# MrTornado24/FENeRF

Measured on AMD Instinct MI355X. Metric: rays/s/GPU forward render (128x128, 24+24 samples, H=256 FiLM-SIREN + 32x96^3 grid), higher is better.
Workload: dtype f16x3 (error-compensated fp16 MFMA, fp32 accumulate; fp32-class accuracy); 1 GPU; configs[1]: CelebA_double_semantic_texture_embedding_256_dim_96 generator, 128x128, 24+24 hierarchical samples, batch 1/GPU, forward-only render, procedural weights; img_size=128, num_steps=24, batch_per_gpu=1

## Files before the change

fenerf_amd/csrc/fenerf_api.cpp:

```cpp
#include <hip/hip_runtime.h>

#include <atomic>
#include <cstddef>
#include <cstdio>
#include <cstdlib>
#include <cstring>
#include <map>
#include <mutex>
#include <new>
#include <string>
#include <vector>

#include "fenerf_internal.h"

namespace fenerf {
static thread_local std::string g_err;
void set_error(const std::string& msg) { g_err = msg; }

static int fail(int code, const std::string& msg) {
  set_error(msg);
  return code;
}
static int hip_fail(hipError_t e, const char* what) {
  return fail(FENERF_E_HIP, std::string(what) + ": " + hipGetErrorString(e));
// ... 159 lines not shown
  {
    std::lock_guard<std::mutex> lock(g_phase_mu);
    recs.swap(g_phase_recs);
  }
  int rc = FENERF_OK;
  for (PhaseRec* r : recs) {
    float t = 0.f;
    hipError_t e = hipEventSynchronize(r->e1);
    if (e == hipSuccess) e = hipEventElapsedTime(&t, r->e0, r->e1);
    if (e == hipSuccess) { ms[r->phase] += (double)t; calls[r->phase] += 1; }
    else rc = hip_fail(e, "fenerf_phase_times");
    (void)hipEventDestroy(r->e0);
    (void)hipEventDestroy(r->e1);
    delete r;
  }
  return rc;
}
extern "C" int fenerf_abi_version(void) { return FENERF_ABI_VERSION; }
static thread_local int g_render_fusion = FENERF_FUSION_AUTO;
static constexpr bool kFusionAutoEnabled = false;
extern "C" int fenerf_set_render_fusion(int mode) {
  const int prev = g_render_fusion;
  g_render_fusion = (mode == FENERF_FUSION_OFF || mode == FENERF_FUSION_FORCE) ? mode : FENERF_FUSION_AUTO;
  return prev;
}
extern "C" int fenerf_set_cu_budget(int cus) {
  const int prev = g_cu_budget;
  g_cu_budget = cus > 0 ? cus : 0;
  return prev;
}

namespace {
struct FieldInfo { const char* name; long offset; };
struct StructInfo { const char* name; long size; const FieldInfo* fields; int n; };
#define FLD(S, f) {#f, (long)offsetof(S, f)}
const FieldInfo kDescFields[] = {
    FLD(FenerfModelDesc, abi_version), FLD(FenerfModelDesc, hidden_dim), FLD(FenerfModelDesc, n_geo), FLD(FenerfModelDesc, n_color),
    FLD(FenerfModelDesc, n_label_layers), FLD(FenerfModelDesc, output_dim), FLD(FenerfModelDesc, grid_ch), FLD(FenerfModelDesc, grid_d),
    FLD(FenerfModelDesc, grid_h), FLD(FenerfModelDesc, grid_w), FLD(FenerfModelDesc, box_scale), FLD(FenerfModelDesc, geo_w),
    FLD(FenerfModelDesc, geo_b), FLD(FenerfModelDesc, color_w), FLD(FenerfModelDesc, color_b), FLD(FenerfModelDesc, label_w),
    FLD(FenerfModelDesc, label_b), FLD(FenerfModelDesc, sigma_w), FLD(FenerfModelDesc, sigma_b), FLD(FenerfModelDesc, rgb_w),
    FLD(FenerfModelDesc, rgb_b), FLD(FenerfModelDesc, grid), FLD(FenerfModelDesc, precision), FLD(FenerfModelDesc, differentiable),
    FLD(FenerfModelDesc, wgrad_bf16_min_points)};
const FieldInfo kOptsFields[] = {
    FLD(FenerfCompositeOpts, clamp_mode), FLD(FenerfCompositeOpts, noise_std), FLD(FenerfCompositeOpts, last_back),
    FLD(FenerfCompositeOpts, white_back), FLD(FenerfCompositeOpts, black_back), FLD(FenerfCompositeOpts, fill_mode),
// ... 851 lines not shown
  p.rows_a = rows_a; p.rows_b = rows_b; p.z_a = z_a; p.z_b = z_b; p.noise = noise; p.o = *opts;
  p.g_rgb = g_rgb; p.d_rows_a = d_rows_a; p.d_rows_b = d_rows_b;
  { PhaseScope ph(PH_COMPOSITE_BWD, stream); return launch_composite_backward(p, merge != 0, stream); }
}

extern "C" size_t fenerf_sparse_select_workspace_bytes(int B, int64_t P) {
  if (B < 1 || P < 1) return 0;
  return sparse_select_workspace_bytes(B, P);
}

extern "C" int fenerf_sparse_select(int B, int R, int N, int C, int64_t cap, const float* d_coarse, const float* d_fine, const float* z_coarse,
                                    const float* z_fine, const float* origins, const float* dirs, const int64_t* images, float* pts, float* rd,
                                    float* d_sel, int32_t* counts, void* workspace, size_t workspace_bytes, void* stream) {
  if (B < 1 || B > 65535 || R < 1 || N < 1 || C < 1 || cap < 1) return fail(FENERF_E_INVALID, "need 1 <= B <= 65535, R, N, C, cap >= 1");
  if ((int64_t)R * N > (int64_t)1 << 36) return fail(FENERF_E_INVALID, "too many samples per image");
  if (!d_coarse || !z_coarse || !origins || !dirs || !pts || !d_sel || !counts || !workspace || (!d_fine) != (!z_fine))
    return fail(FENERF_E_INVALID, "NULL pointer (d_fine and z_fine may be NULL together: one pass)");
  if (workspace_bytes < sparse_select_workspace_bytes(B, (int64_t)R * N)) return fail(FENERF_E_INVALID, "workspace too small (fenerf_sparse_select_workspace_bytes)");
  { PhaseScope ph(PH_OTHER, stream); return launch_sparse_select(B, R, N, C, cap, d_coarse, d_fine, z_coarse, z_fine, origins, dirs, (const long long*)images, pts, rd, d_sel, counts, workspace, stream); }
}

namespace {
struct RenderWs {
  size_t film, coarse, fine, wts, zf, total;
};
RenderWs render_ws(const FenerfModel* m, int B, int R, int N, int hier) {
  RenderWs w;
  const size_t pts = (size_t)B * R * N;
  size_t off = 0;
  w.film = off; off += fenerf_film_workspace_bytes(m, B);
  w.coarse = off; off += align_up(pts * m->C * sizeof(float), 256);
  w.fine = off; off += hier ? align_up(pts * m->C * sizeof(float), 256) : 0;
  w.wts = off; off += hier ? align_up(pts * sizeof(float), 256) : 0;
  w.zf = off; off += hier ? align_up(pts * sizeof(float), 256) : 0;
  w.total = off;
  return w;
}
}

extern "C" size_t fenerf_render_workspace_bytes(const FenerfModel* m, int B, int R, int N, int hierarchical) {
  if (!m || B <= 0 || R <= 0 || N <= 0) return 0;
  return render_ws(m, B, R, N, hierarchical).total;
}

extern "C" int fenerf_render_forward(const FenerfModel* m, int B, int R, int N, int hierarchical, int lock_view,
                                     const float* origins, const float* dirs, const float* z_coarse, const float* u,
                                     const float* noise_coarse, const float* noise_final, const float* freq_geo,
                                     const float* phase_geo, const float* freq_app, const float* phase_app,
                                     const FenerfCompositeOpts* opts, float* out_rgb, float* out_depth,
                                     float* out_weights, float* out_wsum, void* workspace, size_t workspace_bytes,
                                     void* stream) {
  if (!m) return fail(FENERF_E_INVALID, "model is NULL");
  int rc = check_opts(opts);
  if (rc) return rc;
  if (B <= 0 || R <= 0 || N <= 0) return fail(FENERF_E_INVALID, "B, R, N must be > 0");
  const int M = hierarchical ? 2 * N : N;
  if (M > FENERF_MAX_RAY_SAMPLES) return fail(FENERF_E_INVALID, "at most 1024 samples per ray (512 + 512 hierarchical; FENERF_MAX_RAY_SAMPLES)");
// ... 30 lines not shown
    cp.out_ch = out_channels(m->C, opts);
    return run_composite(cp, false, stream);
  }
  float* fine = (float*)(base + ws.fine);
  float* zf = (float*)(base + ws.zf);
  FusedRenderPlan plan;
  if ((g_render_fusion == FENERF_FUSION_FORCE || (g_render_fusion == FENERF_FUSION_AUTO && kFusionAutoEnabled)) &&
      fused_render_plan(m, B, R, N, g_render_fusion == FENERF_FUSION_AUTO, &plan)) {
    CompositeParams c1, c2;
    memset(&c1, 0, sizeof(c1));
    c1.BR = BR; c1.M = N; c1.C = m->C; c1.N = N;
    c1.rows_a = coarse; c1.z_a = z_coarse; c1.noise = noise_coarse;
    c1.o.clamp_mode = opts->clamp_mode; c1.o.noise_std = opts->noise_std;
    c1.sigma_only = 1; c1.out_ch = m->C - 1;
    c1.u = u; c1.z_fine = zf;
    memset(&c2, 0, sizeof(c2));
    c2.BR = BR; c2.M = 2 * N; c2.C = m->C; c2.N = N;
    c2.rows_a = fine; c2.rows_b = coarse; c2.z_a = zf; c2.z_b = z_coarse; c2.noise = noise_final; c2.o = *opts;
    c2.out_rgb = out_rgb; c2.out_depth = out_depth; c2.out_weights = out_weights; c2.out_wsum = out_wsum;
    c2.out_ch = out_channels(m->C, opts);
    sp.out = coarse;
    PhaseScope ph(PH_RENDER_FUSED, stream);
    return launch_render16w_fused(m, sp, plan, zf, fine, c1, c2, stream);
  }
  rc = run_siren(m, sp, stream);
  if (rc) return rc;
  sp.raw_fg = nullptr;
  memset(&cp, 0, sizeof(cp));
  cp.BR = BR; cp.M = N; cp.C = m->C; cp.N = N;
  cp.rows_a = coarse; cp.z_a = z_coarse; cp.noise = noise_coarse;
  cp.o.clamp_mode = opts->clamp_mode; cp.o.noise_std = opts->noise_std;
  cp.sigma_only = 1; cp.out_ch = m->C - 1;
  cp.u = u; cp.z_fine = zf;
  rc = run_composite(cp, false, stream);
  if (rc) return rc;
  sp.z = zf; sp.out = fine;
  rc = run_siren(m, sp, stream);
  if (rc) return rc;
  memset(&cp, 0, sizeof(cp));
  cp.BR = BR; cp.M = 2 * N; cp.C = m->C; cp.N = N;
  cp.rows_a = fine; cp.rows_b = coarse; cp.z_a = zf; cp.z_b = z_coarse; cp.noise = noise_final; cp.o = *opts;
  cp.out_rgb = out_rgb; cp.out_depth = out_depth; cp.out_weights = out_weights; cp.out_wsum = out_wsum;
  cp.out_ch = out_channels(m->C, opts);
  return run_composite(cp, true, stream);
}

// ... 387 lines not shown
```

fenerf_amd/csrc/fenerf_internal.h:

```cpp
#pragma once
#include <cstddef>
#include <cstdint>
#include <map>
#include <mutex>
#include <string>
#include <vector>

#include "../../include/fenerf.h"
#include "fenerf_layout.h"

namespace fenerf {

void set_error(const std::string& msg);
int ensure_dynamic_lds(const void* kfn, size_t bytes);
enum Phase { PH_FILM_PREP = 0, PH_SIREN, PH_SIREN_SAVE, PH_CHAIN, PH_WGRAD_FILM, PH_WGRAD_SQ, PH_WGRAD_SQ_REDUCE, PH_WGRAD_THIN,
             PH_WGRAD_THIN_REDUCE, PH_COMPOSITE, PH_RESAMPLE, PH_COMPOSITE_BWD, PH_REPACK, PH_GRID, PH_RAY_SETUP, PH_OTHER, PH_RENDER_FUSED, PH_COUNT };
static_assert(PH_COUNT == FENERF_N_PHASES, "include/fenerf.h FENERF_N_PHASES");
struct PhaseScope {
  PhaseScope(int phase, void* stream);
  ~PhaseScope();
  void* rec;
};
int launch_cus(const FenerfModel* m);
int check_trig_domain();
// ... 41 lines not shown
  const float* grid;
  int gd, gh, gw;
  float box_scale;
  const float* points;
  const float* pdirs;
  const float* origins;
  const float* dirs;
  const float* z;
  int n_per_ray;
  int lock_view;
  long long P;
  long long pts_per_image;
  float* out;
  long long ring_offset_floats;
  float* tape;
  float* tape_e;
  int tape_format;
  int film_per_point;
  unsigned long long* clk;
  const float* raw_fg; const float* raw_pg; const float* raw_fa; const float* raw_pa;
  const float* film_bias;
  const float* film_inv_scale;
  int n_images;
};

struct SirenBwdParams {
  const float* stream;
  long long ring_offset_floats;
  const float* fp;
  const float* pp;
  long long P, pts_per_image;
  const float* out;
  const float* d_out;
  const float* tape;
  int tape_format;
  float* d_t;
  int bf16_dump;
  float* d_e;
  float* film_tiles;
  const float* points;
  float* d_grid_cl;
  float box_scale;
  int gd, gh, gw;
  int film_per_point;
};

// ... 15 lines not shown
  float* d_rows_a;
  float* d_rows_b;
};

int launch_film_prep(const FenerfModel* m, long long B, const float* fg, const float* pg, const float* fa, const float* pa,
                     float* fp, float* pp, void* stream, bool for_f32_kernel = false,
                     bool twice = false);
int launch_siren(const FenerfModel* m, const SirenParams& p, void* stream);
int launch_siren_f32(const FenerfModel* m, const SirenParams& p, void* stream);
int launch_siren_backward(const FenerfModel* m, const SirenBwdParams& p, void* stream);
int launch_siren_backward16w(const FenerfModel* m, const SirenBwdParams& p, void* stream);
bool use_bf16_dump(const FenerfModel* m, long long total_points);
int bwd16w_film_unit(long long total_points, long long pts_per_image);
size_t wgrad_workspace_bytes(const FenerfModel* m, int B, long long P);
int launch_param_grads(const FenerfModel* m, int B, long long P, const float* points, const float* dirs, const float* fp, const float* pp,
                       const float* out, const float* d_out, const float* tape, const float* tape_e, const float* d_t,
                       const FenerfSirenGrads& g, bool film_only, void* workspace, void* stream, const float* film_tiles = nullptr,
                       int tape_format = 0, const FenerfSirenGrads* weights = nullptr,
                       int film_per_point = 0);
int launch_grid_backward(const FenerfModel* m, long long P, const float* points, const float* d_e, float* d_grid_cl, void* stream);
int launch_siren_input_grads(const FenerfModel* m, int B, long long P, const float* points, const float* fp, const float* d_t, const float* w_geo0,
                             const float* w_color0, int w_color0_ld, float* d_points, float* d_dirs, void* stream);
int launch_siren16w(const FenerfModel* m, const SirenParams& p, void* stream);
struct FusedRenderPlan { int rays_per_group, octs_per_group, blocks; long long groups; };
bool fused_render_plan(const FenerfModel* m, long long B, long long R, int N, bool balanced_only, FusedRenderPlan* plan);
int launch_render16w_fused(const FenerfModel* m, const SirenParams& p, const FusedRenderPlan& plan, float* z_fine, float* out_fine,
                           const CompositeParams& coarse, const CompositeParams& final_, void* stream);
int launch_composite(const CompositeParams& p, bool merge, void* stream);
int launch_composite_backward(const CompositeParams& p, bool merge, void* stream);
int launch_resample(long long BR, int N, const float* z, const float* w, const float* u, float* zf, void* stream);
int launch_sample_pdf(long long BR, int K, int NS, const float* bins, const float* w, const float* u, float* out, void* stream);
int launch_ray_setup(int B, int S, int N, float z_cam, float ray_start, float ray_end, const float* u_jitter,
                     const float* theta, const float* phi, float* origins, float* dirs, float* z, float* pitch, float* yaw,
                     void* stream);
#define FENERF_MULTI_ADD_MAX 64
struct MultiAdd { float* dst[FENERF_MULTI_ADD_MAX]; const float* src[FENERF_MULTI_ADD_MAX]; long long n[FENERF_MULTI_ADD_MAX]; int count; };
struct FilmFold { float* out[4]; const float* in[4]; int row[4]; int B; };
int launch_render_points(int B, int R, int N, long long Pp, const float* origins, const float* dirs, const float* z, float* pts, float* rd, void* stream);
size_t sparse_select_workspace_bytes(int B, long long P);
int launch_sparse_select(int B, int R, int N, int C, long long cap, const float* d_coarse, const float* d_fine, const float* z_coarse,
                         const float* z_fine, const float* origins, const float* dirs, const long long* images, float* pts, float* rd, float* d_sel,
                         int* counts, void* workspace, void* stream);
int launch_pad_rows(const float* src, float* dst, long long nb, long long P, long long Pp, int C, bool to_padded, void* stream);
int launch_multi_add(const MultiAdd& J, void* stream);
int launch_film_fold(const FilmFold& J, void* stream);
int launch_repack(FenerfModel* m, const float* flat, const FenerfRepackMaps* r, float* scale_fwd, float* scale_bwd, void* stream);
// ... 5 lines not shown
```

fenerf_amd/csrc/fenerf_siren_f16w.hip:

```cpp
#include <hip/hip_runtime.h>

#include <type_traits>

#include "fenerf_composite_ray.h"
#include "fenerf_film.h"
#include "fenerf_internal.h"
#include "fenerf_layout.h"
#include "fenerf_trig.h"


namespace fenerf {
namespace w16 {

typedef float f32x4 __attribute__((ext_vector_type(4)));
typedef _Float16 half8 __attribute__((ext_vector_type(8)));
typedef _Float16 half4 __attribute__((ext_vector_type(4)));
typedef _Float16 half2 __attribute__((ext_vector_type(2)));

#define MFMA16W(a, b, c) __builtin_amdgcn_mfma_f32_16x16x32_f16((a), (b), (c), 0, 0, 0)
#define MFMA32W(a, b, c) __builtin_amdgcn_mfma_f32_16x16x4f32((a), (b), (c), 0, 0, 0)

constexpr int CH = FENERF_CH;
constexpr int DPF = FENERF_DPF;
constexpr int NSLOT = FENERF_NSLOT;
// ... 44 lines not shown
}
__device__ __forceinline__ void st_u4_nt(const void* g_uniform, unsigned voff, const u32x4& v) {
  asm volatile("global_store_dwordx4 %0, %1, %2 " FENERF_ST_POLICY "\n\ts_nop 1" : : "v"(voff), "v"(v), "s"(g_uniform) : "memory");
}
struct TapeQ { unsigned q[4]; };
__device__ __forceinline__ unsigned phase_u16(float theta) {
  return __builtin_bit_cast(unsigned, __builtin_fmaf(__builtin_amdgcn_fractf(theta), 65536.f, 8388608.f));
}
#define LDS_FENCE() asm volatile("" ::: "memory")
#ifndef FENERF_WAVE_HALF_COPIES
#define FENERF_WAVE_HALF_COPIES 1
#endif
#ifndef FENERF_EXP_DEPHASE
#define FENERF_EXP_DEPHASE 0
#endif

struct WStream {
  bool skip;
  unsigned long long g_next;
  unsigned voff;
  unsigned ring_lds;
  const char* ring_lane;
  bool early;
};

__device__ __forceinline__ void ws_issue(WStream& w, int slot) {
  const unsigned m0 = w.ring_lds + (unsigned)slot * (CH * 1024);
  if (!w.skip)
    asm volatile(
        "s_mov_b32 m0, %2\n\t"
        "s_nop 0\n\t"
        "global_load_lds_dwordx4 %0, %1"
        :
        : "v"(w.voff), "s"(w.g_next), "s"(m0)
        : "memory");
  w.g_next += CH * 1024;
}

struct AK { float4 hi[2], lo[2]; };
__device__ __forceinline__ void ws_read_lo(AK& a, const WStream& w, int slot, int spl) {
  const float4* p = reinterpret_cast<const float4*>(w.ring_lane + slot * (CH * 1024) + spl * 4096);
  a.lo[0] = p[1 * 64]; a.lo[1] = p[3 * 64];
}
__device__ __forceinline__ void ws_read_hi(AK& a, const WStream& w, int slot, int spl) {
  const float4* p = reinterpret_cast<const float4*>(w.ring_lane + slot * (CH * 1024) + spl * 4096);
  a.hi[0] = p[0 * 64]; a.hi[1] = p[2 * 64];
}
template <bool LO = true>
__device__ __forceinline__ AK ws_read(const WStream& w, int slot, int spl) {
  AK a;
  if (LO) ws_read_lo(a, w, slot, spl);
  else { a.lo[0] = make_float4(0.f, 0.f, 0.f, 0.f); a.lo[1] = a.lo[0]; }
  ws_read_hi(a, w, slot, spl);
  return a;
}

__device__ __forceinline__ void ws_step(WStream& w, int i, bool early) {
  const bool sync = (i & 1) == 0;
  if (sync) {
// ... 107 lines not shown
  constexpr int QBE = QB < 4 ? QB : 4;
  if (qc >= QBE) { p0 = p1 = 0; return; }
  p0 = 4 * qc / QBE;
  p1 = 4 * (qc + 1) / QBE;
}

template <bool FUSED> struct FuseArgs {};
template <> struct FuseArgs<true> {
  int rays_per_group, octs_per_group;
  long long groups, total_rays;
  float* z_fine;
  float* out_fine;
  CompositeParams coarse;
  CompositeParams final_;
};
#ifndef FENERF_EXP_RAY_PHASE
#define FENERF_EXP_RAY_PHASE 2
#endif
#ifndef FENERF_EXP_FUSED_MAXM
#define FENERF_EXP_FUSED_MAXM 128
#endif
constexpr int FUSED_MAXM = FENERF_EXP_FUSED_MAXM;

template <int H, bool GRID, int SAVE, bool FUSED = false, int TERMS2 = 0>
__global__ __launch_bounds__(512, 2) void siren16w_kernel(SirenParams P, int n_geo, int n_color, int n_lab, int C, FuseArgs<FUSED> F) {
  static_assert(!(FUSED && SAVE != 0), "the fused render is the no-grad path");
  static_assert(TERMS2 == 0 || (SAVE == 0 && !FUSED), "the reduced-precision forwards are plain no-grad evaluations");
  constexpr bool LOR = TERMS2 != 1;
  constexpr bool LOC = TERMS2 == 0;
  constexpr int NB = H / 32, KS = H / 32;
  constexpr int QB = (KS + 1) / 2;
  constexpr int C0_KS = KS + (GRID ? 1 : 0) + 1;
  constexpr int C0_QB = (2 * (2 * KS + (GRID ? 2 : 0) + 1) + CH - 1) / CH;
  constexpr int SQ_CHUNKS = pad_stage(NB * QB * CH) / CH;
  constexpr int C0_CHUNKS = pad_stage(NB * C0_QB * CH) / CH;
  constexpr int HEAD_CHUNKS = pad_stage(QB * CH) / CH;
  extern __shared__ __attribute__((aligned(16))) float4 smem[];

  if (P.clk && threadIdx.x == 0) {
    P.clk[(size_t)blockIdx.x * 4 + 0] = __builtin_amdgcn_s_memtime();
    P.clk[(size_t)blockIdx.x * 4 + 1] = __builtin_amdgcn_s_memrealtime();
  }
  const int lane = threadIdx.x & 63;
  const int wave = __builtin_amdgcn_readfirstlane(threadIdx.x >> 6);
  const int n = lane & 15, g = lane >> 4;
  const int L = n_geo + n_color;
  const int stage_f4 = (16 * C + 3) / 4;
  char* lds = reinterpret_cast<char*>(smem);
  char* ring = lds;
  constexpr int FILM_F = H * 4 < 1024 ? 1024 : H * 4;
// ... 17 lines not shown
    constexpr int NW = (int)(sizeof(CompositeParams) / 4);
    static_assert(sizeof(CompositeParams) % 4 == 0 && NW <= 256, "copied one dword per thread");
    const int t = threadIdx.x & 255;
    const unsigned* src = reinterpret_cast<const unsigned*>(threadIdx.x < 256 ? &F.coarse : &F.final_);
    if (t < NW) reinterpret_cast<unsigned*>(ray_par + (threadIdx.x >> 8))[t] = src[t];
  }
  WAIT_VMCNT(0);
  __syncthreads();

  WStream ws;
  {
    const int spl = wave >> 2, rt = (wave >> 1) & 1, hl = wave & 1;
    const int gi = n >> 2, r = n & 3;
    const int row = 16 * (gi >> 1) + 4 * (gi & 1) + 8 * rt + r;
    const int e_old = 2 * (2 * spl + (g >> 1)) + hl;
    ws.voff = e_old * 1024 + ((g & 1) * 32 + row) * 16;
  }
  const unsigned long long g_stream = reinterpret_cast<unsigned long long>(P.stream + P.ring_offset_floats);
  ws.g_next = g_stream;
  ws.ring_lds = __builtin_amdgcn_readfirstlane(lds_addr(ring) + wave * 1024);
  ws.ring_lane = ring + lane * 16;
  ws.early = wave < NWAVE / 2;
  ws.skip = TERMS2 == 1 && (wave & 1);

  const long long ntiles = (P.P + 15) / 16;
  const long long nocts = (ntiles + NWAVE - 1) / NWAVE;
  int opg = 1;
  long long nunits = nocts;
  if constexpr (FUSED) { opg = F.octs_per_group; nunits = F.groups; }
  const int nblk = gridDim.x;
  const int nx = nblk < 8 ? nblk : 8;
  const int xcd = blockIdx.x % nx, bi = blockIdx.x / nx;
  const int blocks_in_x = nblk / nx + (xcd < nblk % nx ? 1 : 0);
  const long long o_begin = nunits * xcd / nx, o_end = nunits * (xcd + 1) / nx;

  if (P.raw_fg && o_begin + bi < o_end) {
    const long long p_first = (o_begin + bi) * opg * (NWAVE * 16);
    long long p_last = o_end * opg * (NWAVE * 16) - 1;
    if (p_last >= P.P) p_last = P.P - 1;
    film_prep_prologue(P, p_first / P.pts_per_image, p_last / P.pts_per_image, H, n_geo, n_color);
  }

#pragma unroll
  for (int i = 0; i < DPF; ++i) ws_issue(ws, i);
  WAIT_VMCNT(DPF - 1);
  __builtin_amdgcn_s_barrier();
  LDS_FENCE();
  if (wave >= NWAVE / 2) __builtin_amdgcn_s_setprio(1);
  APipe a_cur;
  a_cur.c = ws_read<LOR>(ws, 0, 0);
  a_cur.n = ws_read<LOR>(ws, 0, 1);


  for (long long unit = o_begin + bi; unit < o_end; unit += blocks_in_x) {
  const int nsub = FUSED ? 2 * opg : 1;
#pragma unroll 1
  for (int sub = 0; sub < nsub; ++sub) {
    const bool fine_pass = FUSED && sub >= opg;
    const long long oct = FUSED ? unit * opg + (fine_pass ? sub - opg : sub) : unit;
    const float* z_src = P.z;
    float* out_dst = P.out;
    if constexpr (FUSED) {
      if (fine_pass) { z_src = F.z_fine; out_dst = F.out_fine; }
    }
    ws.g_next = g_stream + (unsigned long long)DPF * (CH * 1024);
    const long long tile = oct * NWAVE + wave;
    long long pt = tile * 16 + n;
    if (pt >= P.P) pt = P.P - 1;
    const long long img = __builtin_amdgcn_readfirstlane((int)(pt / P.pts_per_image));
    float px, py, pz, dx, dy, dz;
    if (P.points) {
      px = P.points[pt * 3 + 0]; py = P.points[pt * 3 + 1]; pz = P.points[pt * 3 + 2];
      if (P.pdirs) { dx = P.pdirs[pt * 3 + 0]; dy = P.pdirs[pt * 3 + 1]; dz = P.pdirs[pt * 3 + 2]; }
      else { dx = 0.f; dy = 0.f; dz = -1.f; }
    } else {
      const long long ray = pt / P.n_per_ray;
      const float zz = z_src[pt];
      const float ox = P.origins[ray * 3 + 0], oy = P.origins[ray * 3 + 1], oz = P.origins[ray * 3 + 2];
      dx = P.dirs[ray * 3 + 0]; dy = P.dirs[ray * 3 + 1]; dz = P.dirs[ray * 3 + 2];
      px = __fadd_rn(ox, __fmul_rn(dx, zz)); py = __fadd_rn(oy, __fmul_rn(dy, zz)); pz = __fadd_rn(oz, __fmul_rn(dz, zz));
      if (P.lock_view) { dx = 0.f; dy = 0.f; dz = -1.f; }
    }
    const float qx = px * P.box_scale, qy = py * P.box_scale, qz = pz * P.box_scale;
    constexpr int TL = SAVE == 2 ? H * 64 : H * 128;
    const int tile_odd = (int)(tile & 1);
    const char* tape_tile = SAVE ? uniform_ptr(reinterpret_cast<const char*>(P.tape) + (size_t)(tile >> 1) * L * TL) : nullptr;
    auto tape_of = [&](int layer) {
      TapeW<SAVE> t{SAVE ? uniform_ptr(tape_tile + (size_t)layer * TL) : nullptr};
      if (SAVE) asm volatile("s_nop 4" ::: "memory");
      return t;
    };

    const float* fp_img = P.fp + (size_t)img * L * H;
    const float* pp_img = P.pp + (size_t)img * L * H;
    auto film_issue = [&](int layer) {
      const unsigned dst = __builtin_amdgcn_readfirstlane(lds_addr(film_base) + (layer & 1) * FILM_BYTES);
      const float* gf = fp_img + (size_t)layer * H;
      const float* gp = pp_img + (size_t)layer * H;
      const unsigned vo = (unsigned)opaque(lane) * 16;
      for (int off = 0; off < H * 4; off += 1024) {
        glds_1k_s(reinterpret_cast<const char*>(gf) + off, vo, dst + off);
        glds_1k_s(reinterpret_cast<const char*>(gp) + off, vo, dst + FILM_F + off);
      }
    };
    film_issue(0);
    if (L > 1) film_issue(1);

    float e[8];
#pragma unroll
    for (int i = 0; i < 8; ++i) e[i] = 0.f;
    if (GRID) {
      const int ch0 = 16 * (g & 1) + 8 * (g >> 1);
      const float ix = ((qx + 1.f) / 2.f) * (float)(P.gw - 1);
      const float iy = ((qy + 1.f) / 2.f) * (float)(P.gh - 1);
      const float iz = ((qz + 1.f) / 2.f) * (float)(P.gd - 1);
      const float x0 = floorf(ix), y0 = floorf(iy), z0 = floorf(iz);
#pragma unroll
      for (int c = 0; c < 8; ++c) {
        const int cz = c >> 2, cy = (c >> 1) & 1, cx = c & 1;
        const float xi = x0 + cx, yi = y0 + cy, zi = z0 + cz;
        const float wx = cx ? (ix - x0) : (x0 + 1.f - ix);
        const float wy = cy ? (iy - y0) : (y0 + 1.f - iy);
        const float wz = cz ? (iz - z0) : (z0 + 1.f - iz);
        const float wgt = wx * wy * wz;
        const bool ok = xi >= 0.f && xi <= (float)(P.gw - 1) && yi >= 0.f && yi <= (float)(P.gh - 1) && zi >= 0.f &&
                        zi <= (float)(P.gd - 1);
        if (ok) {
          const long long vox = ((long long)(int)zi * P.gh + (int)yi) * P.gw + (int)xi;
          const float4* gp = reinterpret_cast<const float4*>(P.grid + vox * 32 + ch0);
#pragma unroll
          for (int q = 0; q < 2; ++q) {
            const float4 v = gp[q];
            e[4 * q + 0] += v.x * wgt; e[4 * q + 1] += v.y * wgt; e[4 * q + 2] += v.z * wgt; e[4 * q + 3] += v.w * wgt;
          }
        }
      }
    }
    if (SAVE && GRID) {
      float4* ep = reinterpret_cast<float4*>(P.tape_e + pt * 32 + 16 * (g & 1) + 8 * (g >> 1));
      ep[0] = make_float4(e[0], e[1], e[2], e[3]);
      ep[1] = make_float4(e[4], e[5], e[6], e[7]);
    }
    {
      half8 eh, el, dh, dl;
#pragma unroll
      for (int t = 0; t < 8; ++t) {
        const float v = e[t] * F16_ACT_SCALE;
        const _Float16 hh = (_Float16)v;
        eh[t] = hh; el[t] = (_Float16)(v - (float)hh);
      }
      const float d3[3] = {dx * F16_ACT_SCALE, dy * F16_ACT_SCALE, dz * F16_ACT_SCALE};
#pragma unroll
      for (int t = 0; t < 8; ++t) { dh[t] = (_Float16)0.f; dl[t] = (_Float16)0.f; }
#pragma unroll
      for (int t = 0; t < 3; ++t) {
        const float v = g == 0 ? d3[t] : 0.f;
        const _Float16 hh = (_Float16)v;
        dh[t] = hh; dl[t] = (_Float16)(v - (float)hh);
      }
      float4* ext = ext_wave + lane;
      ext[0] = __builtin_bit_cast(float4, eh); ext[64] = __builtin_bit_cast(float4, el);
      ext[128] = __builtin_bit_cast(float4, dh); ext[192] = __builtin_bit_cast(float4, dl);
    }
    WAIT_VMCNT(0);
    LDS_FENCE();

    auto film_lane = [&](int layer) -> const float* {
      const int gq = opaque(lane) >> 4;
      return reinterpret_cast<const float*>(film_base + (layer & 1) * FILM_BYTES) + 16 * (gq >> 1) + 4 * (gq & 1);
    };

    half8 xh[KS], xl[KS];
    {
      const float b = g == 0 ? qx : (g == 1 ? qy : (g == 2 ? qz : 0.f));
      const int gi = n >> 2, r = n & 3;
      const float* wl = l0_lds + ((g & 1) * 32 + 16 * (gi >> 1) + 4 * (gi & 1) + r) * 4 + (g >> 1);
      const TapeW<SAVE> tw0 = tape_of(0);
#pragma unroll
      for (int nb = 0; nb < NB; ++nb) {
        f32x4 acc[2];
#pragma unroll
        for (int rt = 0; rt < 2; ++rt) {
          const f32x4 z4 = {0.f, 0.f, 0.f, 0.f};
          acc[rt] = MFMA32W(wl[nb * 256 + 8 * rt * 4], b, z4);
        }
        epi_all<KS, FILM_F / 4, SAVE>(acc, nb, film_lane(0), xh, xl, tw0, tile_odd);
      }
    }
    auto film_layer = [&](auto ph_c, int l) {
      constexpr int PH = decltype(ph_c)::value;
      const float* ff = film_lane(l);
      const TapeW<SAVE> tw = tape_of(l);
      half8 yh[KS], yl[KS];
      if (l + 1 < L) film_issue(l + 1);
      if (SQ_CHUNKS < DPF + 2) WAIT_VMCNT(0);
      if (l == n_geo) {
        const float4* ext = ext_wave + opaque(lane);
        auto bop0 = [&](int sp, half8& bh, half8& bl) -> bool {
          if (sp < KS) { bh = xh[sp]; bl = xl[sp]; return true; }
          if (GRID && sp == KS) { bh = as_half8(ext[0]); bl = as_half8(ext[64]); return true; }
          if (sp == C0_KS - 1) { bh = as_half8(ext[128]); bl = as_half8(ext[192]); return true; }
          return false;
        };
        f32x4 acc_prev[2] = {{0.f, 0.f, 0.f, 0.f}, {0.f, 0.f, 0.f, 0.f}};
        TapeQ tq;
#pragma unroll
        for (int nb = 0; nb < NB; ++nb) {
          f32x4 acc[2] = {{0.f, 0.f, 0.f, 0.f}, {0.f, 0.f, 0.f, 0.f}};
#pragma unroll
          for (int qc = 0; qc < C0_QB; ++qc) {
            chunk_step<LOR, LOC, PH>(acc, a_cur, ws, nb * C0_QB + qc, 2 * qc, bop0, [&](FilmQ2& fq) {
              if (nb > 0) {
                int p0, p1;
                piece_range<C0_QB>(qc, p0, p1);
#pragma unroll
                for (int pc = 0; pc < 4; ++pc)
                  if (pc >= p0 && pc < p1) fq.q[pc] = epi_load<FILM_F / 4>(nb - 1, pc, ff);
              }
            }, [&](const FilmQ2& fq) {
              if (nb > 0) {
                int p0, p1;
                piece_range<C0_QB>(qc, p0, p1);
#pragma unroll
                for (int pc = 0; pc < 4; ++pc)
                  if (pc >= p0 && pc < p1) epi_compute<KS, SAVE>(acc_prev, nb - 1, pc, fq.q[pc], yh, yl, tw, tile_odd, tq);
              }
            });
          }
          acc_prev[0] = acc[0]; acc_prev[1] = acc[1];
        }
#pragma unroll
        for (int i = NB * C0_QB; i < C0_CHUNKS; ++i) chunk_skip<LOR, PH>(a_cur, ws, i);
        epi_all<KS, FILM_F / 4, SAVE>(acc_prev, NB - 1, ff, yh, yl, tw, tile_odd);
        {
          f32x4 acc[2] = {{0.f, 0.f, 0.f, 0.f}, {0.f, 0.f, 0.f, 0.f}};
          auto bop = [&](int sp, half8& bh, half8& bl) -> bool {
            if (sp < KS) { bh = xh[sp]; bl = xl[sp]; return true; }
            return false;
          };
#pragma unroll
          for (int qc = 0; qc < QB; ++qc) chunk_step<LOR, true, PH>(acc, a_cur, ws, qc, 2 * qc, bop, [](FilmQ2&) {}, [](const FilmQ2&) {});
#pragma unroll
          for (int i = QB; i < HEAD_CHUNKS; ++i) chunk_skip<LOR, PH>(a_cur, ws, i);
          const int lane_o = opaque(lane);
          const int n_o = lane_o & 15, f_o = 16 * (lane_o >> 5) + 4 * ((lane_o >> 4) & 1);
#pragma unroll
          for (int rt = 0; rt < 2; ++rt) {
#pragma unroll
            for (int r = 0; r < 4; ++r) {
              const int row = f_o + 8 * rt + r;
              if (row <= n_lab) {
                const int ch = row < n_lab ? row : C - 1;
                stage[n_o * C + ch] = acc[rt][r] * cst[row] + cst[32 + row];
              }
            }
          }
        }
// ... 21 lines not shown
              }
            }, [&](const FilmQ2& fq) {
              if (nb > 0) {
                int p0, p1;
                piece_range<QB>(qc, p0, p1);
#pragma unroll
                for (int pc = 0; pc < 4; ++pc)
                  if (pc >= p0 && pc < p1) epi_compute<KS, SAVE>(acc_prev, nb - 1, pc, fq.q[pc], yh, yl, tw, tile_odd, tq);
              }
            });
          }
          acc_prev[0] = acc[0]; acc_prev[1] = acc[1];
        }
#pragma unroll
        for (int i = NB * QB; i < SQ_CHUNKS; ++i) chunk_skip<LOR, PH>(a_cur, ws, i);
        epi_all<KS, FILM_F / 4, SAVE>(acc_prev, NB - 1, ff, yh, yl, tw, tile_odd);
        };
        if constexpr (TERMS2 == 2) {
          if (l < n_geo) square_stage(std::true_type{}); else square_stage(std::false_type{});
        } else {
          square_stage(std::integral_constant<bool, LOR>{});
        }
      }
#pragma unroll
      for (int k = 0; k < KS; ++k) { xh[k] = yh[k]; xl[k] = yl[k]; }
    };
#pragma unroll 1
    for (int l = 1; l < L; ++l) {
#if FENERF_WAVE_HALF_COPIES
      if (ws.early) film_layer(std::integral_constant<int, 0>{}, l); else film_layer(std::integral_constant<int, 1>{}, l);
#else
      film_layer(std::integral_constant<int, -1>{}, l);
#endif
    }
    {
      constexpr int PH = -1;
      f32x4 acc[2] = {{0.f, 0.f, 0.f, 0.f}, {0.f, 0.f, 0.f, 0.f}};
      auto bop = [&](int sp, half8& bh, half8& bl) -> bool {
        if (sp < KS) { bh = xh[sp]; bl = xl[sp]; return true; }
        return false;
      };
#pragma unroll
      for (int qc = 0; qc < QB; ++qc) chunk_step<LOR, LOC, PH>(acc, a_cur, ws, qc, 2 * qc, bop, [](FilmQ2&) {}, [](const FilmQ2&) {});
#pragma unroll
      for (int i = QB; i < HEAD_CHUNKS; ++i) chunk_skip<LOR, PH>(a_cur, ws, i);
      const int lane_o = opaque(lane);
      const int n_o = lane_o & 15;
      if ((lane_o >> 4) == 0) {
#pragma unroll
        for (int r = 0; r < 3; ++r) {
          const float v = acc[0][r] * cst[64 + r] + cst[68 + r];
          stage[n_o * C + (C - 4) + r] = 1.f / (1.f + __expf(-v));
        }
      }
    }
    __builtin_amdgcn_fence(__ATOMIC_RELEASE, "wavefront");
    __builtin_amdgcn_wave_barrier();
    __builtin_amdgcn_fence(__ATOMIC_ACQUIRE, "wavefront");
    {
      const long long base = tile * 16 * C;
      const long long limit = P.P * C;
      for (int i = opaque(lane); i < 16 * C; i += 64)
        if (base + i < limit) out_dst[base + i] = stage[i];
    }
    WAIT_VMCNT(0);
    __builtin_amdgcn_wave_barrier();
    if constexpr (FUSED) {
      if (FENERF_EXP_RAY_PHASE > 0 && (sub == opg - 1 || sub == nsub - 1)) {
        __builtin_amdgcn_fence(__ATOMIC_RELEASE, "workgroup");
        __builtin_amdgcn_s_barrier();
        __builtin_amdgcn_fence(__ATOMIC_ACQUIRE, "workgroup");
        float* sc = reinterpret_cast<float*>(ext_wave);
        float* s_z = sc;
        float* s_zs = sc + FUSED_MAXM;
        int* s_ord = reinterpret_cast<int*>(sc + 2 * FUSED_MAXM + 4);
        float* s_w = sc + 3 * FUSED_MAXM + 4;
        const int lane_r = opaque(lane);
        const long long ray0 = unit * F.rays_per_group;
        for (int r = wave; r < F.rays_per_group; r += NWAVE) {
          const long long ray = ray0 + r;
          if (FENERF_EXP_RAY_PHASE > 1 && ray < F.total_rays) {
#pragma unroll 1
            for (int rep = 0; rep < (FENERF_EXP_RAY_PHASE > 2 ? 2 : 1); ++rep) {
              if (!fine_pass) composite_ray<false, FUSED_MAXM>(ray_par[0], ray, lane_r, s_z, s_zs, s_ord, s_w);
              else composite_ray<true, FUSED_MAXM>(ray_par[1], ray, lane_r, s_z, s_zs, s_ord, s_w);
              __builtin_amdgcn_wave_barrier();
            }
          }
          __builtin_amdgcn_wave_barrier();
        }
        if (!fine_pass) {
          __builtin_amdgcn_fence(__ATOMIC_RELEASE, "workgroup");
          __builtin_amdgcn_s_barrier();
          __builtin_amdgcn_fence(__ATOMIC_ACQUIRE, "workgroup");
        }
        WAIT_VMCNT(0);
      }
    }
  }
  }
  WAIT_VMCNT(0);
  __builtin_amdgcn_s_barrier();
  if (P.clk && threadIdx.x == 0) {
    P.clk[(size_t)blockIdx.x * 4 + 2] = __builtin_amdgcn_s_memtime();
    P.clk[(size_t)blockIdx.x * 4 + 3] = __builtin_amdgcn_s_memrealtime();
  }
}

static int hip_fail16w(hipError_t e, const char* what) {
  set_error(std::string(what) + ": " + hipGetErrorString(e));
  return FENERF_E_HIP;
}

static size_t lds_bytes_16w(const FenerfModel* m, int H) {
  const int stage_f4 = (16 * m->C + 3) / 4;
  const size_t film_f = H * 4 < 1024 ? 1024 : H * 4;
  return (size_t)NSLOT * CH * 1024 + (size_t)NWAVE * 2 * (2 * film_f) + (size_t)(H / 32) * 1024 + 80 * 4 +
         (size_t)NWAVE * stage_f4 * 16 + (size_t)NWAVE * 4096;
}

template <int H, bool GRID>
static int launch_fused_t(const FenerfModel* m, const SirenParams& p, const FuseArgs<true>& F, int blocks, void* stream) {
  const size_t lds = lds_bytes_16w(m, H) + (2 * sizeof(CompositeParams) + 255) / 256 * 256;
  auto kfn = siren16w_kernel<H, GRID, 0, true>;
  if (int rc = ensure_dynamic_lds(reinterpret_cast<const void*>(kfn), lds)) return rc;
  hipLaunchKernelGGL(kfn, dim3((unsigned)blocks), dim3(512), lds, (hipStream_t)stream, p, m->n_geo, m->n_color, m->n_lab, m->C, F);
  hipError_t e = hipGetLastError();
  return e == hipSuccess ? FENERF_OK : hip_fail16w(e, "fused render launch");
}

template <int H, bool GRID, int SAVE, int TERMS2 = 0>
static int launch_t(const FenerfModel* m, const SirenParams& p, void* stream) {
  const size_t lds = lds_bytes_16w(m, H);
  auto kfn = siren16w_kernel<H, GRID, SAVE, false, TERMS2>;
  if (int rc = ensure_dynamic_lds(reinterpret_cast<const void*>(kfn), lds)) return rc;
  const long long ntiles = (p.P + 15) / 16;
  long long blocks = (ntiles + NWAVE - 1) / NWAVE;
  if (blocks > m->num_cus) blocks = m->num_cus;
  if (blocks < 1) blocks = 1;
  hipLaunchKernelGGL(kfn, dim3((unsigned)blocks), dim3(512), lds, (hipStream_t)stream, p, m->n_geo, m->n_color, m->n_lab, m->C, FuseArgs<false>{});
  hipError_t e = hipGetLastError();
  return e == hipSuccess ? FENERF_OK : hip_fail16w(e, "siren16w launch");
}

}

static int launch_siren16w_one(const FenerfModel* m, const SirenParams& q, void* stream) {
  const bool g = m->grid_ch != 0;
  if (q.tape && q.tape_format == FENERF_TAPE_U16) {
    switch (m->H) {
      case 32: return g ? w16::launch_t<32, true, 2>(m, q, stream) : w16::launch_t<32, false, 2>(m, q, stream);
      case 64: return g ? w16::launch_t<64, true, 2>(m, q, stream) : w16::launch_t<64, false, 2>(m, q, stream);
      case 96: return g ? w16::launch_t<96, true, 2>(m, q, stream) : w16::launch_t<96, false, 2>(m, q, stream);
      case 128: return g ? w16::launch_t<128, true, 2>(m, q, stream) : w16::launch_t<128, false, 2>(m, q, stream);
      case 192: return g ? w16::launch_t<192, true, 2>(m, q, stream) : w16::launch_t<192, false, 2>(m, q, stream);
      case 256: return g ? w16::launch_t<256, true, 2>(m, q, stream) : w16::launch_t<256, false, 2>(m, q, stream);
    }
  }
  if (q.tape) {
    switch (m->H) {
      case 32: return g ? w16::launch_t<32, true, 1>(m, q, stream) : w16::launch_t<32, false, 1>(m, q, stream);
      case 64: return g ? w16::launch_t<64, true, 1>(m, q, stream) : w16::launch_t<64, false, 1>(m, q, stream);
      case 96: return g ? w16::launch_t<96, true, 1>(m, q, stream) : w16::launch_t<96, false, 1>(m, q, stream);
      case 128: return g ? w16::launch_t<128, true, 1>(m, q, stream) : w16::launch_t<128, false, 1>(m, q, stream);
      case 192: return g ? w16::launch_t<192, true, 1>(m, q, stream) : w16::launch_t<192, false, 1>(m, q, stream);
      case 256: return g ? w16::launch_t<256, true, 1>(m, q, stream) : w16::launch_t<256, false, 1>(m, q, stream);
    }
  }
  if (m->forward_mode == FENERF_FORWARD_F16X2) {
    switch (m->H) {
      case 32: return g ? w16::launch_t<32, true, 0, 1>(m, q, stream) : w16::launch_t<32, false, 0, 1>(m, q, stream);
      case 64: return g ? w16::launch_t<64, true, 0, 1>(m, q, stream) : w16::launch_t<64, false, 0, 1>(m, q, stream);
      case 96: return g ? w16::launch_t<96, true, 0, 1>(m, q, stream) : w16::launch_t<96, false, 0, 1>(m, q, stream);
      case 128: return g ? w16::launch_t<128, true, 0, 1>(m, q, stream) : w16::launch_t<128, false, 0, 1>(m, q, stream);
      case 192: return g ? w16::launch_t<192, true, 0, 1>(m, q, stream) : w16::launch_t<192, false, 0, 1>(m, q, stream);
      case 256: return g ? w16::launch_t<256, true, 0, 1>(m, q, stream) : w16::launch_t<256, false, 0, 1>(m, q, stream);
    }
  }
  if (m->forward_mode == FENERF_FORWARD_F16X3_COLOR_X2) {
    switch (m->H) {
      case 32: return g ? w16::launch_t<32, true, 0, 2>(m, q, stream) : w16::launch_t<32, false, 0, 2>(m, q, stream);
      case 64: return g ? w16::launch_t<64, true, 0, 2>(m, q, stream) : w16::launch_t<64, false, 0, 2>(m, q, stream);
      case 96: return g ? w16::launch_t<96, true, 0, 2>(m, q, stream) : w16::launch_t<96, false, 0, 2>(m, q, stream);
      case 128: return g ? w16::launch_t<128, true, 0, 2>(m, q, stream) : w16::launch_t<128, false, 0, 2>(m, q, stream);
      case 192: return g ? w16::launch_t<192, true, 0, 2>(m, q, stream) : w16::launch_t<192, false, 0, 2>(m, q, stream);
      case 256: return g ? w16::launch_t<256, true, 0, 2>(m, q, stream) : w16::launch_t<256, false, 0, 2>(m, q, stream);
    }
  }
  switch (m->H) {
    case 32: return g ? w16::launch_t<32, true, 0>(m, q, stream) : w16::launch_t<32, false, 0>(m, q, stream);
    case 64: return g ? w16::launch_t<64, true, 0>(m, q, stream) : w16::launch_t<64, false, 0>(m, q, stream);
    case 96: return g ? w16::launch_t<96, true, 0>(m, q, stream) : w16::launch_t<96, false, 0>(m, q, stream);
    case 128: return g ? w16::launch_t<128, true, 0>(m, q, stream) : w16::launch_t<128, false, 0>(m, q, stream);
    case 192: return g ? w16::launch_t<192, true, 0>(m, q, stream) : w16::launch_t<192, false, 0>(m, q, stream);
    case 256: return g ? w16::launch_t<256, true, 0>(m, q, stream) : w16::launch_t<256, false, 0>(m, q, stream);
  }
  set_error("unsupported hidden_dim");
  return FENERF_E_UNSUPPORTED;
}

bool fused_render_plan(const FenerfModel* m, long long B, long long R, int N, bool balanced_only, FusedRenderPlan* plan) {
  if (m->precision != FENERF_PREC_F16X3 || N < 3 || 2 * N > w16::FUSED_MAXM) return false;
  if (m->forward_mode != FENERF_FORWARD_F16X3) return false;
  int g = N, b = 128;
  while (b) { const int t = g % b; g = b; b = t; }
  const int G = 128 / g, opg = N / g;
  if (R % G != 0) return false;
  const long long groups = B * R / G, nocts = groups * opg;
  const long long cus = launch_cus(m);
  const long long blocks_f = groups < cus ? groups : cus, blocks_p = nocts < cus ? nocts : cus;
  if (balanced_only && (groups + blocks_f - 1) / blocks_f * opg > (nocts + blocks_p - 1) / blocks_p) return false;
  plan->rays_per_group = G; plan->octs_per_group = opg; plan->groups = groups; plan->blocks = (int)blocks_f;
  return true;
}

int launch_render16w_fused(const FenerfModel* m, const SirenParams& p, const FusedRenderPlan& plan, float* z_fine, float* out_fine,
                           const CompositeParams& coarse, const CompositeParams& final_, void* stream) {
  w16::FuseArgs<true> F;
  F.rays_per_group = plan.rays_per_group; F.octs_per_group = plan.octs_per_group; F.groups = plan.groups;
  F.total_rays = coarse.BR;
  F.z_fine = z_fine; F.out_fine = out_fine; F.coarse = coarse; F.final_ = final_;
// ... 46 lines not shown
```

Baseline: 6.113 million rays/s.

## Defer colour branch to compacted queue of points with positive density

Adds a deferred-colour mode to the fp16x3 SIREN forward. The trunk layers run for every point, and only points with positive sigma keep their trunk activations, which go into a per-block global queue. A separate colour pass then runs the grid sample, colour FiLM layers and RGB head on full compacted tiles. The weight stream is rerouted with jump addresses so that each pass loads only the layers it uses. The goal is to skip colour-branch work for empty-space samples, paid for with queue traffic, extra barriers and a second weight stream, and it relies on zero-density points not needing RGB under relu clamping.

```diff
diff --git a/fenerf_amd/csrc/fenerf_api.cpp b/fenerf_amd/csrc/fenerf_api.cpp
--- a/fenerf_amd/csrc/fenerf_api.cpp
+++ b/fenerf_amd/csrc/fenerf_api.cpp
@@ -205,6 +205,18 @@
 extern "C" int fenerf_set_render_fusion(int mode) {
   const int prev = g_render_fusion;
   g_render_fusion = (mode == FENERF_FUSION_OFF || mode == FENERF_FUSION_FORCE) ? mode : FENERF_FUSION_AUTO;
+  return prev;
+}
+static thread_local bool g_deferred_colour = true;
+static thread_local int g_deferred_colour_renders = 0;
+extern "C" int fenerf_internal_deferred_colour(int mode) {
+  if (mode == 2) {
+    const int n = g_deferred_colour_renders;
+    g_deferred_colour_renders = 0;
+    return n;
+  }
+  const int prev = g_deferred_colour ? 0 : 1;
+  g_deferred_colour = mode != 1;
   return prev;
 }
 extern "C" int fenerf_set_cu_budget(int cus) {
@@ -1102,7 +1114,7 @@
 
 namespace {
 struct RenderWs {
-  size_t film, coarse, fine, wts, zf, total;
+  size_t film, coarse, fine, wts, zf, dq, total;
 };
 RenderWs render_ws(const FenerfModel* m, int B, int R, int N, int hier) {
   RenderWs w;
@@ -1113,6 +1125,7 @@
   w.fine = off; off += hier ? align_up(pts * m->C * sizeof(float), 256) : 0;
   w.wts = off; off += hier ? align_up(pts * sizeof(float), 256) : 0;
   w.zf = off; off += hier ? align_up(pts * sizeof(float), 256) : 0;
+  w.dq = off; off += hier && m->precision == FENERF_PREC_F16X3 ? align_up(siren16w_defer_queue_bytes(m), 256) : 0;
   w.total = off;
   return w;
 }
@@ -1189,6 +1202,11 @@
     sp.out = coarse;
     PhaseScope ph(PH_RENDER_FUSED, stream);
     return launch_render16w_fused(m, sp, plan, zf, fine, c1, c2, stream);
+  }
+  if (g_deferred_colour && m->precision == FENERF_PREC_F16X3 && m->forward_mode == FENERF_FORWARD_F16X3 && opts->clamp_mode == FENERF_CLAMP_RELU &&
+      !noise_final && !opts->last_back && m->n_geo >= 2 && BR * N <= 0x7fffffffLL) {
+    sp.defer_q = base + ws.dq;
+    ++g_deferred_colour_renders;
   }
   rc = run_siren(m, sp, stream);
   if (rc) return rc;
diff --git a/fenerf_amd/csrc/fenerf_internal.h b/fenerf_amd/csrc/fenerf_internal.h
--- a/fenerf_amd/csrc/fenerf_internal.h
+++ b/fenerf_amd/csrc/fenerf_internal.h
@@ -87,6 +87,7 @@
   const float* film_bias;
   const float* film_inv_scale;
   int n_images;
+  char* defer_q;
 };
 
 struct SirenBwdParams {
@@ -148,6 +149,7 @@
 int launch_siren_input_grads(const FenerfModel* m, int B, long long P, const float* points, const float* fp, const float* d_t, const float* w_geo0,
                              const float* w_color0, int w_color0_ld, float* d_points, float* d_dirs, void* stream);
 int launch_siren16w(const FenerfModel* m, const SirenParams& p, void* stream);
+size_t siren16w_defer_queue_bytes(const FenerfModel* m);
 struct FusedRenderPlan { int rays_per_group, octs_per_group, blocks; long long groups; };
 bool fused_render_plan(const FenerfModel* m, long long B, long long R, int N, bool balanced_only, FusedRenderPlan* plan);
 int launch_render16w_fused(const FenerfModel* m, const SirenParams& p, const FusedRenderPlan& plan, float* z_fine, float* out_fine,
diff --git a/fenerf_amd/csrc/fenerf_siren_f16w.hip b/fenerf_amd/csrc/fenerf_siren_f16w.hip
--- a/fenerf_amd/csrc/fenerf_siren_f16w.hip
+++ b/fenerf_amd/csrc/fenerf_siren_f16w.hip
@@ -90,6 +90,8 @@
   unsigned ring_lds;
   const char* ring_lane;
   bool early;
+  bool jmp;
+  unsigned long long j0f, j0t, j1f, j1t;
 };
 
 __device__ __forceinline__ void ws_issue(WStream& w, int slot) {
@@ -103,6 +105,10 @@
         : "v"(w.voff), "s"(w.g_next), "s"(m0)
         : "memory");
   w.g_next += CH * 1024;
+  if (w.jmp) {
+    if (w.g_next == w.j0f) w.g_next = w.j0t;
+    else if (w.g_next == w.j1f) w.g_next = w.j1t;
+  }
 }
 
 struct AK { float4 hi[2], lo[2]; };
@@ -256,10 +262,13 @@
 #endif
 constexpr int FUSED_MAXM = FENERF_EXP_FUSED_MAXM;
 
-template <int H, bool GRID, int SAVE, bool FUSED = false, int TERMS2 = 0>
+constexpr int DQ_CAP = 256;
+
+template <int H, bool GRID, int SAVE, bool FUSED = false, int TERMS2 = 0, bool DEFER = false>
 __global__ __launch_bounds__(512, 2) void siren16w_kernel(SirenParams P, int n_geo, int n_color, int n_lab, int C, FuseArgs<FUSED> F) {
   static_assert(!(FUSED && SAVE != 0), "the fused render is the no-grad path");
   static_assert(TERMS2 == 0 || (SAVE == 0 && !FUSED), "the reduced-precision forwards are plain no-grad evaluations");
+  static_assert(!DEFER || (SAVE == 0 && !FUSED && TERMS2 == 0), "deferred colour is a mode of the plain no-grad forward");
   constexpr bool LOR = TERMS2 != 1;
   constexpr bool LOC = TERMS2 == 0;
   constexpr int NB = H / 32, KS = H / 32;
@@ -323,6 +332,8 @@
   ws.ring_lane = ring + lane * 16;
   ws.early = wave < NWAVE / 2;
   ws.skip = TERMS2 == 1 && (wave & 1);
+  ws.jmp = DEFER;
+  ws.j0f = ws.j0t = ws.j1f = ws.j1t = 0;
 
   const long long ntiles = (P.P + 15) / 16;
   const long long nocts = (ntiles + NWAVE - 1) / NWAVE;
@@ -352,6 +363,15 @@
   a_cur.c = ws_read<LOR>(ws, 0, 0);
   a_cur.n = ws_read<LOR>(ws, 0, 1);
 
+  constexpr unsigned long long CHB = CH * 1024;
+  const unsigned long long s_c0 = g_stream + (unsigned long long)(n_geo - 1) * SQ_CHUNKS * CHB;
+  const unsigned long long s_head = s_c0 + (unsigned long long)C0_CHUNKS * CHB;
+  const unsigned long long s_col = s_head + (unsigned long long)HEAD_CHUNKS * CHB;
+  char* const q_x = DEFER ? P.defer_q + (size_t)blockIdx.x * DQ_CAP * (KS * 128 + 4) : nullptr;
+  int* const q_pt = reinterpret_cast<int*>(q_x + (size_t)2 * KS * DQ_CAP * 64);
+  int* const q_waves = reinterpret_cast<int*>(cst + 72);
+  int q_head = 0, q_cnt = 0;
+  long long q_img = 0;
 
   for (long long unit = o_begin + bi; unit < o_end; unit += blocks_in_x) {
   const int nsub = FUSED ? 2 * opg : 1;
@@ -364,11 +384,31 @@
     if constexpr (FUSED) {
       if (fine_pass) { z_src = F.z_fine; out_dst = F.out_fine; }
     }
-    ws.g_next = g_stream + (unsigned long long)DPF * (CH * 1024);
     const long long tile = oct * NWAVE + wave;
+    half8 xh[KS], xl[KS];
+    bool trunk_pass = true, from_queue = false, keep_own = false;
+    int n_take = 0;
+#pragma unroll 1
+    for (;;) {
+    if (!DEFER || trunk_pass) {
+      ws.g_next = g_stream + (unsigned long long)DPF * (CH * 1024);
+      if (DEFER) { ws.j0f = s_c0; ws.j0t = s_head; ws.j1f = s_col; ws.j1t = g_stream; }
+    }
     long long pt = tile * 16 + n;
+    const bool real = pt < P.P;
     if (pt >= P.P) pt = P.P - 1;
-    const long long img = __builtin_amdgcn_readfirstlane((int)(pt / P.pts_per_image));
+    long long img = __builtin_amdgcn_readfirstlane((int)(pt / P.pts_per_image));
+    bool write_rgb = true;
+    if (DEFER && !trunk_pass) {
+      if (from_queue) {
+        const int j = 16 * wave + n;
+        write_rgb = j < n_take;
+        pt = write_rgb ? (long long)q_pt[(q_head + j) & (DQ_CAP - 1)] : q_img * P.pts_per_image;
+        img = q_img;
+      } else {
+        write_rgb = keep_own;
+      }
+    }
     float px, py, pz, dx, dy, dz;
     if (P.points) {
       px = P.points[pt * 3 + 0]; py = P.points[pt * 3 + 1]; pz = P.points[pt * 3 + 2];
@@ -404,13 +444,29 @@
         glds_1k_s(reinterpret_cast<const char*>(gp) + off, vo, dst + FILM_F + off);
       }
     };
-    film_issue(0);
-    if (L > 1) film_issue(1);
+    const bool colour_pass = !DEFER || !trunk_pass;
+    if (DEFER && !trunk_pass) {
+      film_issue(n_geo);
+    } else {
+      film_issue(0);
+      if (L > 1) film_issue(1);
+    }
+    if (DEFER && !trunk_pass && from_queue) {
+      const int lq = opaque(lane);
+      const int e = (q_head + 16 * wave + (lq & 15)) & (DQ_CAP - 1);
+      const float4* qs = reinterpret_cast<const float4*>(q_x + (size_t)e * 64 + (lq >> 4) * 16);
+      const float4 z4 = make_float4(0.f, 0.f, 0.f, 0.f);
+#pragma unroll
+      for (int k = 0; k < KS; ++k) {
+        xh[k] = as_half8(write_rgb ? qs[(size_t)(2 * k) * DQ_CAP * 4] : z4);
+        xl[k] = as_half8(write_rgb ? qs[(size_t)(2 * k + 1) * DQ_CAP * 4] : z4);
+      }
+    }
 
     float e[8];
 #pragma unroll
     for (int i = 0; i < 8; ++i) e[i] = 0.f;
-    if (GRID) {
+    if (GRID && colour_pass) {
       const int ch0 = 16 * (g & 1) + 8 * (g >> 1);
       const float ix = ((qx + 1.f) / 2.f) * (float)(P.gw - 1);
       const float iy = ((qy + 1.f) / 2.f) * (float)(P.gh - 1);
@@ -442,7 +498,7 @@
       ep[0] = make_float4(e[0], e[1], e[2], e[3]);
       ep[1] = make_float4(e[4], e[5], e[6], e[7]);
     }
-    {
+    if (colour_pass) {
       half8 eh, el, dh, dl;
 #pragma unroll
       for (int t = 0; t < 8; ++t) {
@@ -465,14 +521,19 @@
     }
     WAIT_VMCNT(0);
     LDS_FENCE();
+    if (DEFER && !trunk_pass) {
+      __builtin_amdgcn_s_barrier();
+      LDS_FENCE();
+      a_cur.c = ws_read<LOR>(ws, 0, 0);
+      a_cur.n = ws_read<LOR>(ws, 0, 1);
+    }
 
     auto film_lane = [&](int layer) -> const float* {
       const int gq = opaque(lane) >> 4;
       return reinterpret_cast<const float*>(film_base + (layer & 1) * FILM_BYTES) + 16 * (gq >> 1) + 4 * (gq & 1);
     };
 
-    half8 xh[KS], xl[KS];
-    {
+    if (!DEFER || trunk_pass) {
       const float b = g == 0 ? qx : (g == 1 ? qy : (g == 2 ? qz : 0.f));
       const int gi = n >> 2, r = n & 3;
       const float* wl = l0_lds + ((g & 1) * 32 + 16 * (gi >> 1) + 4 * (gi & 1) + r) * 4 + (g >> 1);
@@ -493,9 +554,10 @@
       const float* ff = film_lane(l);
       const TapeW<SAVE> tw = tape_of(l);
       half8 yh[KS], yl[KS];
-      if (l + 1 < L) film_issue(l + 1);
+      if (l + 1 < ((DEFER && trunk_pass) ? n_geo : L)) film_issue(l + 1);
       if (SQ_CHUNKS < DPF + 2) WAIT_VMCNT(0);
       if (l == n_geo) {
+        if (!DEFER || !trunk_pass) {
         const float4* ext = ext_wave + opaque(lane);
         auto bop0 = [&](int sp, half8& bh, half8& bl) -> bool {
           if (sp < KS) { bh = xh[sp]; bl = xl[sp]; return true; }
@@ -533,7 +595,8 @@
 #pragma unroll
         for (int i = NB * C0_QB; i < C0_CHUNKS; ++i) chunk_skip<LOR, PH>(a_cur, ws, i);
         epi_all<KS, FILM_F / 4, SAVE>(acc_prev, NB - 1, ff, yh, yl, tw, tile_odd);
-        {
+        }
+        if (!DEFER || trunk_pass) {
           f32x4 acc[2] = {{0.f, 0.f, 0.f, 0.f}, {0.f, 0.f, 0.f, 0.f}};
           auto bop = [&](int sp, half8& bh, half8& bl) -> bool {
             if (sp < KS) { bh = xh[sp]; bl = xl[sp]; return true; }
@@ -601,18 +664,26 @@
           square_stage(std::integral_constant<bool, LOR>{});
         }
       }
-#pragma unroll
-      for (int k = 0; k < KS; ++k) { xh[k] = yh[k]; xl[k] = yl[k]; }
+      if (!DEFER || !trunk_pass || l != n_geo) {
+#pragma unroll
+        for (int k = 0; k < KS; ++k) { xh[k] = yh[k]; xl[k] = yl[k]; }
+      }
     };
 #pragma unroll 1
-    for (int l = 1; l < L; ++l) {
+    for (int l = (DEFER && !trunk_pass) ? n_geo : 1; l < ((DEFER && trunk_pass) ? n_geo + 1 : L); ++l) {
 #if FENERF_WAVE_HALF_COPIES
       if (ws.early) film_layer(std::integral_constant<int, 0>{}, l); else film_layer(std::integral_constant<int, 1>{}, l);
 #else
       film_layer(std::integral_constant<int, -1>{}, l);
 #endif
     }
-    {
+    if (!colour_pass) {
+      const int lane_o = opaque(lane);
+      if ((lane_o >> 4) == 0) {
+#pragma unroll
+        for (int r = 0; r < 3; ++r) stage[(lane_o & 15) * C + (C - 4) + r] = 0.f;
+      }
+    } else {
       constexpr int PH = -1;
       f32x4 acc[2] = {{0.f, 0.f, 0.f, 0.f}, {0.f, 0.f, 0.f, 0.f}};
       auto bop = [&](int sp, half8& bh, half8& bl) -> bool {
@@ -629,14 +700,16 @@
 #pragma unroll
         for (int r = 0; r < 3; ++r) {
           const float v = acc[0][r] * cst[64 + r] + cst[68 + r];
-          stage[n_o * C + (C - 4) + r] = 1.f / (1.f + __expf(-v));
+          const float s = 1.f / (1.f + __expf(-v));
+          if (!DEFER) stage[n_o * C + (C - 4) + r] = s;
+          else if (write_rgb) out_dst[pt * C + (C - 4) + r] = s;
         }
       }
     }
     __builtin_amdgcn_fence(__ATOMIC_RELEASE, "wavefront");
     __builtin_amdgcn_wave_barrier();
     __builtin_amdgcn_fence(__ATOMIC_ACQUIRE, "wavefront");
-    {
+    if (!DEFER || trunk_pass) {
       const long long base = tile * 16 * C;
       const long long limit = P.P * C;
       for (int i = opaque(lane); i < 16 * C; i += 64)
@@ -676,6 +749,74 @@
         WAIT_VMCNT(0);
       }
     }
+    if constexpr (!DEFER) {
+      break;
+    } else {
+      bool in_place = false;
+      if (trunk_pass) {
+        const int lk = opaque(lane);
+        const float sig = stage[(lk & 15) * C + (C - 1)];
+        const bool kept = real && !(sig <= 0.f);
+        const unsigned m16 = (unsigned)__ballot(kept) & 0xFFFFu;
+        if (lk == 0) q_waves[wave] = __builtin_popcount(m16);
+        __builtin_amdgcn_fence(__ATOMIC_RELEASE, "workgroup");
+        __builtin_amdgcn_s_barrier();
+        __builtin_amdgcn_fence(__ATOMIC_ACQUIRE, "workgroup");
+        int tot = 0, pre = 0;
+#pragma unroll
+        for (int w = 0; w < NWAVE; ++w) {
+          const int c = q_waves[w];
+          tot += c;
+          pre += w < wave ? c : 0;
+        }
+        tot = __builtin_amdgcn_readfirstlane(tot);
+        pre = __builtin_amdgcn_readfirstlane(pre);
+        const long long p0 = oct * (NWAVE * 16);
+        const long long p1 = p0 + NWAVE * 16 - 1 < P.P ? p0 + NWAVE * 16 - 1 : P.P - 1;
+        const long long img0 = p0 / P.pts_per_image;
+        keep_own = kept;
+        in_place = img0 != p1 / P.pts_per_image || (q_cnt == 0 && tot == NWAVE * 16);
+        if (!in_place && tot > 0) {
+          if (q_cnt == 0) q_img = img0;
+          if (kept) {
+            const int e = (q_head + q_cnt + pre + __builtin_popcount(m16 & ((1u << (lk & 15)) - 1u))) & (DQ_CAP - 1);
+            float4* qd = reinterpret_cast<float4*>(q_x + (size_t)e * 64 + (lk >> 4) * 16);
+#pragma unroll
+            for (int k = 0; k < KS; ++k) {
+              qd[(size_t)(2 * k) * DQ_CAP * 4] = __builtin_bit_cast(float4, xh[k]);
+              qd[(size_t)(2 * k + 1) * DQ_CAP * 4] = __builtin_bit_cast(float4, xl[k]);
+            }
+            if ((lk >> 4) == 0) q_pt[e] = (int)pt;
+          }
+          q_cnt += tot;
+        }
+      } else if (from_queue) {
+        q_head = (q_head + n_take) & (DQ_CAP - 1);
+        q_cnt -= n_take;
+      }
+      const long long nxt = unit + blocks_in_x;
+      const bool flush = nxt >= o_end || nxt * (NWAVE * 16) / P.pts_per_image != q_img;
+      if (in_place) {
+        from_queue = false;
+      } else if (q_cnt >= NWAVE * 16) {
+        from_queue = true; n_take = NWAVE * 16;
+      } else if (q_cnt > 0 && flush) {
+        from_queue = true; n_take = q_cnt;
+      } else {
+        break;
+      }
+      trunk_pass = false;
+      asm volatile("s_waitcnt lgkmcnt(0)" ::: "memory");
+      WAIT_VMCNT(0);
+      __builtin_amdgcn_fence(__ATOMIC_RELEASE, "workgroup");
+      __builtin_amdgcn_s_barrier();
+      __builtin_amdgcn_fence(__ATOMIC_ACQUIRE, "workgroup");
+      ws.j0f = s_head; ws.j0t = s_col; ws.j1f = 0; ws.j1t = 0;
+      ws.g_next = s_c0;
+#pragma unroll
+      for (int i = 0; i < DPF; ++i) ws_issue(ws, i);
+    }
+    }
   }
   }
   WAIT_VMCNT(0);
@@ -708,10 +849,10 @@
   return e == hipSuccess ? FENERF_OK : hip_fail16w(e, "fused render launch");
 }
 
-template <int H, bool GRID, int SAVE, int TERMS2 = 0>
+template <int H, bool GRID, int SAVE, int TERMS2 = 0, bool DEFER = false>
 static int launch_t(const FenerfModel* m, const SirenParams& p, void* stream) {
   const size_t lds = lds_bytes_16w(m, H);
-  auto kfn = siren16w_kernel<H, GRID, SAVE, false, TERMS2>;
+  auto kfn = siren16w_kernel<H, GRID, SAVE, false, TERMS2, DEFER>;
   if (int rc = ensure_dynamic_lds(reinterpret_cast<const void*>(kfn), lds)) return rc;
   const long long ntiles = (p.P + 15) / 16;
   long long blocks = (ntiles + NWAVE - 1) / NWAVE;
@@ -746,6 +887,16 @@
       case 256: return g ? w16::launch_t<256, true, 1>(m, q, stream) : w16::launch_t<256, false, 1>(m, q, stream);
     }
   }
+  if (q.defer_q) {
+    switch (m->H) {
+      case 32: return g ? w16::launch_t<32, true, 0, 0, true>(m, q, stream) : w16::launch_t<32, false, 0, 0, true>(m, q, stream);
+      case 64: return g ? w16::launch_t<64, true, 0, 0, true>(m, q, stream) : w16::launch_t<64, false, 0, 0, true>(m, q, stream);
+      case 96: return g ? w16::launch_t<96, true, 0, 0, true>(m, q, stream) : w16::launch_t<96, false, 0, 0, true>(m, q, stream);
+      case 128: return g ? w16::launch_t<128, true, 0, 0, true>(m, q, stream) : w16::launch_t<128, false, 0, 0, true>(m, q, stream);
+      case 192: return g ? w16::launch_t<192, true, 0, 0, true>(m, q, stream) : w16::launch_t<192, false, 0, 0, true>(m, q, stream);
+      case 256: return g ? w16::launch_t<256, true, 0, 0, true>(m, q, stream) : w16::launch_t<256, false, 0, 0, true>(m, q, stream);
+    }
+  }
   if (m->forward_mode == FENERF_FORWARD_F16X2) {
     switch (m->H) {
       case 32: return g ? w16::launch_t<32, true, 0, 1>(m, q, stream) : w16::launch_t<32, false, 0, 1>(m, q, stream);
@@ -776,6 +927,10 @@
   }
   set_error("unsupported hidden_dim");
   return FENERF_E_UNSUPPORTED;
+}
+
+size_t siren16w_defer_queue_bytes(const FenerfModel* m) {
+  return (size_t)m->num_cus * w16::DQ_CAP * ((size_t)(m->H / 32) * 128 + 4);
 }
 
 bool fused_render_plan(const FenerfModel* m, long long B, long long R, int N, bool balanced_only, FusedRenderPlan* plan) {
```

Result: slower. 5.856 million rays/s, median of 2 (-4.2%).
